# matyasosvath/hutoken

Hardware: AMD Instinct MI355X
Metric: GB/s input text encoded (GPT-2 vocab) at 1/2/4/8 GPUs; bit-exact ids (higher is better)
Workload: dtype u8

## Files before the change

hutoken_amd/csrc/hutk_kernels.hip:

```cpp
#include <hip/hip_runtime.h>

#include <type_traits>

#include "hutk_kdev.h"
#include "hutk_lab.h"

namespace hutk {

__device__ __noinline__ void cut_note_cold(uint32_t* noreal_bits, uint32_t* counters, uint32_t tile, unsigned long long mine,
                                                  uint32_t last16, uint32_t* cutpos) {
    if ((threadIdx.x & 63) != 0) return;
    if (mine == 0) {
        atomicOr(&noreal_bits[tile >> 5], 1u << (tile & 31));
        atomicAdd(&counters[CTR_NOREAL_TILES], 1u);
    } else {
        *cutpos = 1u + (uint32_t)(16 * (63 - __builtin_clzll(mine)) + 31 - __builtin_clz(last16 & 0xFFFFu));
    }
}

struct Win8 { uint32_t d[8]; };
__device__ __noinline__ uint32_t classify16_exact_cold(Win8 w, uint32_t dbits, uint32_t* tmp) {
#pragma unroll
    for (int i = 0; i < 8; i++) tmp[i] = w.d[i];
    return classify16_exact(*reinterpret_cast<const uint32_t(*)[8]>(tmp), dbits);
// ... 161 lines not shown
            if (X.arena_ws[a] == ws) return X.arena_n[a];
        int n = 0;
        for (int i = 0; i < nb; i++) n += !is_cont(X.sb[ws + LOOKBACK + i]);
        return n;
    };
    static_assert(LOOKBACK + TILE_BYTES + 3 + 4 * (wc::KEY_DWORDS + 1) <= WINDOW, "key reads inside the window");
    [[maybe_unused]] auto wc_key = [&](const Tile& X, int ws, int nb, uint32_t (&k)[wc::KEY_DWORDS]) {
        const int a = (ws + LOOKBACK) & ~3, o8 = 8 * ((ws + LOOKBACK) & 3);
        const uint32_t* sw = reinterpret_cast<const uint32_t*>(X.sb + a);
        uint32_t q[wc::KEY_DWORDS + 1];
#pragma unroll
        for (int j = 0; j <= wc::KEY_DWORDS; j++) q[j] = sw[j];
#pragma unroll
        for (int j = 0; j < wc::KEY_DWORDS; j++) k[j] = funnel_r(q[j + 1], q[j], o8);
        wc::make_key(k, nb);
    };
    [[maybe_unused]] bool learn_open = false;
    [[maybe_unused]] const uint32_t wc_shard = blockIdx.x & (wc::LIST_SHARDS - 1u), wc_shard_cap = W.wc_list_cap / wc::LIST_SHARDS;
    if constexpr (WCACHE && !ONE) {
        if (T.wc_on && W.wc_list_cap) {
            const uint32_t cnt = __hip_atomic_load(&T.wc_ctl[wc::ctl_count(wc_shard)], __ATOMIC_RELAXED, __HIP_MEMORY_SCOPE_AGENT);
            const uint32_t closed = __hip_atomic_load(&T.wc_ctl[wc::CTL_CLOSED], __ATOMIC_RELAXED, __HIP_MEMORY_SCOPE_AGENT);
            learn_open = __builtin_amdgcn_readfirstlane((int)(cnt < wc_shard_cap && closed == 0)) != 0;
        }
    }
    const int64_t t0 = tile * TILE_BYTES;
    const int64_t gw = t0 - LOOKBACK;
    const uint32_t* wmask32 = reinterpret_cast<const uint32_t*>(wmask16);
    const int64_t tile_end = (t0 + TILE_BYTES < A.n_bytes) ? t0 + TILE_BYTES : A.n_bytes;
    int64_t dfirst = 0;
    if constexpr (ONE) {
        if (threadIdx.x == 0) { *A.err = 0; W.noreal_bits[0] = 0; }
        if (threadIdx.x < N_COUNTERS) W.counters[threadIdx.x] = 0;
        if (A.status)
            for (int64_t d = threadIdx.x; d < A.n_docs; d += 64 * WAVES) A.status[d] = 0;
        if (tile_ok) {
            int64_t cnt = 0;
            for (int64_t d0 = 0; d0 <= A.n_docs; d0 += 64) {
                const int64_t d = d0 + lane;
                cnt += __popcll(__ballot(d <= A.n_docs && A.offsets[d] < gw));
            }
            dfirst = cnt;
            if (lane == 0) W.tile_first_doc[tile] = cnt;
        }
    } else {
        dfirst = tile_ok ? W.tile_first_doc[tile] : 0;
    }
    uint32_t own = 0;
    static_assert(WINDOW / 16 > 64 && WINDOW / 16 <= 128, "two chunks per lane");
    const bool whole = tile_ok && gw >= 0 && gw + WINDOW <= A.n_bytes;
    uint4 pre0 = make_uint4(0, 0, 0, 0), pre1 = pre0;
    if (whole) {
        pre0 = *reinterpret_cast<const uint4*>(A.bytes + gw + 16 * lane);
        if (lane < WINDOW / 16 - 64) pre1 = *reinterpret_cast<const uint4*>(A.bytes + gw + 16 * (lane + 64));
    }
    constexpr int DFA_CHUNKS = (dfa::TABLE_BYTES + 256) / 16;
    static_assert(DFA_CHUNKS <= 2 * 64 * WAVES || WAVES < 4, "two chunks of the automaton's table per thread");
    uint4 dfa0 = make_uint4(0, 0, 0, 0), dfa1 = dfa0;
    if (WAVES >= 4) {
        if ((int)threadIdx.x < DFA_CHUNKS) dfa0 = T.split_dfa[threadIdx.x];
        if ((int)threadIdx.x + 64 * WAVES < DFA_CHUNKS) dfa1 = T.split_dfa[threadIdx.x + 64 * WAVES];
    }
    int64_t pre_o = 0;
    if (tile_ok && !A.first_bits && dfirst + lane <= A.n_docs) pre_o = A.offsets[dfirst + lane];
    if (WAVES >= 4) {
        if ((int)threadIdx.x < DFA_CHUNKS) reinterpret_cast<uint4*>(&s_m.c)[threadIdx.x] = dfa0;
        if ((int)threadIdx.x + 64 * WAVES < DFA_CHUNKS) reinterpret_cast<uint4*>(&s_m.c)[threadIdx.x + 64 * WAVES] = dfa1;
    } else {
        for (int i = threadIdx.x; i < DFA_CHUNKS; i += 64 * WAVES) reinterpret_cast<uint4*>(&s_m.c)[i] = T.split_dfa[i];
    }
    if (!BYTE_MODE) {
        for (int i = threadIdx.x; i < 256; i += 64 * WAVES) {
            s_item_sym[i] = Sym<SymT>::narrow(T.item_sym[i]);
            const unsigned long long direct = __ballot(T.item_direct[i] != 0);
            if (lane == 0) {
                s_item_direct[i >> 5] = (uint32_t)direct;
                s_item_direct[(i >> 5) + 1] = (uint32_t)(direct >> 32);
            }
        }
    }
    if (threadIdx.x == 0) s_exc_cnt = 0;
    __syncthreads();
    uint32_t my_exc_off = 0;
    if (tile_ok) {
        HUTK_STAMP(0);

        if (whole) {
            *reinterpret_cast<uint4*>(sb + 16 * lane) = pre0;
            if (lane < WINDOW / 16 - 64) *reinterpret_cast<uint4*>(sb + 16 * (lane + 64)) = pre1;
        } else
        for (int c = lane; c < WINDOW / 16; c += 64) {
            const int64_t p = gw + 16 * c;
            if (p >= 0 && p + 16 <= A.n_bytes) {
                *reinterpret_cast<uint4*>(sb + 16 * c) = *reinterpret_cast<const uint4*>(A.bytes + p);
            } else {
                for (int k = 0; k < 16; k++) {
                    const int64_t q = p + k;
                    sb[16 * c + k] = (q >= 0 && q < A.n_bytes) ? A.bytes[q] : (uint8_t)0;
                }
            }
        }
        if (lane < WINDOW / 32 + 3) docm[lane] = 0;
        if (lane < NPOS / 32 + 2) { mergem[lane] = 0; excm[lane] = 0; livem[lane] = 0; }
        if (lane == 0) { s_arena_used = 0; s_extra = 0; me.cutpos = 0; }
        if (lane < ARENA_WORDS) { arena_ws[lane] = 0xFFFFu; arena_live[lane] = 0; }
        if (lane < 8) wmask16[64 + lane] = 0xFFFFu;
        wave_sync();

        if (A.first_bits) {
            if (lane < WINDOW / 32) {
                const int64_t g = gw + 32 * lane;
                const int64_t w = g >> 5;
                const uint32_t lo = w >= 0 ? A.first_bits[w] : 0u, hi = A.first_bits[w + 1];
                docm[lane] = (lo >> 16) | (hi << 16);
            }
        } else
        for (int64_t d = dfirst + lane; d <= A.n_docs; d += 64) {
            const int64_t o = d == dfirst + lane ? pre_o : A.offsets[d];
            if (o >= gw + WINDOW) break;
            const int li = (int)(o - gw);
            if (li >= 0) atomicOr(&docm[li >> 5], 1u << (li & 31));
        }
        wave_sync();
        HUTK_STAMP(1);

        const int kb = LOOKBACK + 16 * lane;
        Win w;
        {
            const uint64_t* src = reinterpret_cast<const uint64_t*>(sb + kb - 8);
            w.a = src[0]; w.b = src[1]; w.c = src[2]; w.d = src[3];
        }
        const uint32_t dbits = (uint32_t)bits64(docm, kb - 8);
        uint32_t flags;
        unsigned long long with_start;
        uint32_t last_real16;
        {
            const uint32_t dw[8] = {(uint32_t)w.a, (uint32_t)(w.a >> 32), (uint32_t)w.b, (uint32_t)(w.b >> 32),
                                    (uint32_t)w.c, (uint32_t)(w.c >> 32), (uint32_t)w.d, (uint32_t)(w.d >> 32)};
            bool exotic;
            if (A.word_bits) {
                flags = reinterpret_cast<const uint16_t*>(A.word_bits)[(t0 >> 4) + lane];
                exotic = false;
            } else {
                flags = classify16_dfa(dw, dbits, reinterpret_cast<const uint16_t*>(s_m.c.dfa), s_m.c.lut,
                                       &exotic);
            }
            if (exotic) {
                Win8 w8;
    #pragma unroll
                for (int i = 0; i < 8; i++) w8.d[i] = dw[i];
                flags = classify16_exact_cold(w8, dbits, reinterpret_cast<uint32_t*>(S) + 8 * lane);
            }
            with_start = __ballot(flags != 0);
            last_real16 = (uint32_t)__builtin_amdgcn_readlane((int)flags, 63 - __builtin_clzll((with_start & 0x0FFFFFFFFFFFFFFFull) | 1ull));
            if (T.seam_on && !A.word_bits) {
                const uint64_t K8 = 0x8080808080808080ull;
                uint64_t m0 = w.b & (w.b << 1) & (w.b << 2) & K8;
                uint64_t m1 = w.c & (w.c << 1) & (w.c << 2) & K8;
                if (m0 | m1) {
                    const uint64_t p0 = (w.b << 8) | (w.a >> 56), p1 = (w.c << 8) | (w.b >> 56);
                    for (; m0; m0 &= m0 - 1) {
                        const int sh = __builtin_ctzll(m0) - 7;
                        const uint32_t y = (uint32_t)(w.b >> sh) & 0xFFu, x = (uint32_t)(p0 >> sh) & 0xFFu;
                        const uint32_t sm = *reinterpret_cast<const uint32_t*>(s_m.c.dfa + dfa::seam_offset(x));
                        bool join = (sm >> (y & 31u)) & 1u;
                        if (!join) flags |= 1u << (sh >> 3);
                    }
                    for (; m1; m1 &= m1 - 1) {
                        const int sh = __builtin_ctzll(m1) - 7;
                        const uint32_t y = (uint32_t)(w.c >> sh) & 0xFFu, x = (uint32_t)(p1 >> sh) & 0xFFu;
                        const uint32_t sm = *reinterpret_cast<const uint32_t*>(s_m.c.dfa + dfa::seam_offset(x));
                        bool join = (sm >> (y & 31u)) & 1u;
                        if (!join) flags |= 1u << (8 + (sh >> 3));
                    }
                }
            }
        }
        {
            const int64_t valid = tile_end - (t0 + 16 * lane);
            const uint64_t lo = w.b, hi = w.c;
            const uint64_t K1 = 0x0101010101010101ull, K8 = 0x8080808080808080ull;
            uint64_t zlo = (lo - K1) & ~lo & K8, zhi = (hi - K1) & ~hi & K8;
            if (valid < 16) {
                const int v = valid < 0 ? 0 : (int)valid;
                zlo &= v >= 8 ? ~0ull : ((1ull << (8 * v)) - 1ull);
                zhi &= v <= 8 ? 0ull : ((1ull << (8 * (v - 8))) - 1ull);
            }
            if (zlo | zhi) raise(A.err, HUTK_E_NUL_BYTE);
        }
        {
            const unsigned long long sb_ = __ballot((flags & 0xFFFFu) != 0);
            const int l0 = sb_ ? __builtin_ctzll(sb_) : 0;
            const uint32_t f0 = (uint32_t)__builtin_amdgcn_readlane((int)flags, l0) & 0xFFFFu;
            if (lane == 0 && tile_ok) W.tile_first_start[tile] = sb_ ? (uint32_t)(16 * l0 + __builtin_ctz(f0)) : 0xFFFFu;
        }
        wmask16[lane] = (uint16_t)flags;
#if HUTK_PERTURB_VALU
        {
            uint32_t x = flags | 1u;
            for (int i = 0; i < HUTK_PERTURB_VALU / 4; i++) {
                x ^= x << 13; x ^= x >> 17;
                asm volatile("" : "+v"(x));
            }
            if (x == 0x9E3779B9u) raise(A.err, HUTK_E_MEMORY);
        }
#endif
        HUTK_STAMP(2);

        wave_sync();
        HUTK_STAMP(3);

        const int limit = (int)(tile_end - t0);
        own = flags;
        {
            const int lo = 16 * lane;
            if (lo >= limit) own = 0;
            else if (lo + 16 > limit) own &= (1u << (limit - lo)) - 1u;
        }
        if (!A.word_bits || !A.gap_bits) {
            const unsigned long long mine = with_start & ((1ull << ((limit + 15) >> 4)) - 1ull);
            if (mine == 0 || (with_start >> 60) == 0)
                cut_note_cold(W.noreal_bits, W.counters, (uint32_t)tile, mine, last_real16, &me.cutpos);
        }
        reinterpret_cast<uint16_t*>(livem)[lane] = (uint16_t)own;
        uint32_t rest = own;
        if constexpr (BYTE_MODE && !MULTI) {
            if (!A.word_bits && ONE) {
                constexpr int WORD_KEY = sizeof(SymT) == 2 ? WORD_KEY_BYTES_16 : WORD_KEY_BYTES_32;
                constexpr int KSH = sizeof(SymT) == 2 ? 16 : 32;
                const uint32_t f32 = flags | ((uint32_t)wmask16[lane + 1] << 16);
                uint32_t x = f32 >> 1;
                x |= x >> 1;
                x |= x >> 2;
                x |= x >> 4;
                x |= x >> (WORD_KEY - 8);
                uint32_t shorts = own & x;
                if (T.has_prefix) shorts &= ~(uint32_t)bits64(docm, 16 * lane + LOOKBACK);
                rest = own & ~shorts;
                uint32_t nS;
                uint32_t sidx = wave_excl_scan(__popc(shorts), lane, &nS);
                for (uint32_t r0 = 0; r0 < nS; r0 += 64) {
                    while (shorts && sidx - r0 < 64u) {
                        stage[sidx - r0] = (uint16_t)(16 * lane + __builtin_ctz(shorts));
                        shorts &= shorts - 1;
                        sidx++;
                    }
                    wave_sync();
                    if (r0 + lane < nS) {
                        const uint32_t ws = stage[lane];
                        uint32_t wb;
                        __builtin_memcpy(&wb, reinterpret_cast<const uint8_t*>(wmask16) + ((ws + 1u) >> 3), 4);
                        const uint32_t nb = 1u + (uint32_t)__builtin_ctz(wb >> ((ws + 1u) & 7u));
                        uint4 key;
                        __builtin_memcpy(&key, sb + LOOKBACK + ws, 16);
                        const uint32_t isym = T.item_sym[key.x & 0xFFu];
                        const uint64_t mlo = nb >= 8 ? ~0ull : ((1ull << (8 * nb)) - 1ull);
                        const uint64_t mhi = nb <= 8 ? 0ull : ((1ull << (8 * (nb - 8))) - 1ull);
                        const uint32_t k0 = key.x & (uint32_t)mlo, k1 = key.y & (uint32_t)(mlo >> 32);
                        const uint32_t k2 = key.z & (uint32_t)mhi, k3 = key.w & (uint32_t)(mhi >> 32);
                        bool done = nb == 1;
                        uint32_t sym = isym;
                        if (T.word_mask) {
                            const uint32_t wh = word_hash(k0, k1, k2, k3);
                            uint4 s1 = reinterpret_cast<const uint4*>(T.word_tab)[wh & T.word_mask];
                            uint4 s2 = reinterpret_cast<const uint4*>(T.word_tab)[word_slot2(wh, T.word_mask)];
                            asm volatile("" : "+v"(s1.x), "+v"(s2.x));
                            const uint32_t d1 = KSH == 32 ? 0u : (s1.w ^ k3) << (KSH & 31);
                            const uint32_t d2 = KSH == 32 ? 0u : (s2.w ^ k3) << (KSH & 31);
                            const bool hit1 = ((s1.x ^ k0) | (s1.y ^ k1) | (s1.z ^ k2) | d1) == 0;
                            const bool hit2 = ((s2.x ^ k0) | (s2.y ^ k1) | (s2.z ^ k2) | d2) == 0;
                            if (nb != 1 && (hit1 || hit2)) {
                                const uint32_t swd = hit1 ? s1.w : s2.w;
                                sym = KSH == 32 ? swd : swd >> (KSH & 31);
                                done = true;
                            }
                        }
                        if (done) {
                            S[ws] = Sym<SymT>::narrow(sym);
                        } else {
                            atomicOr(&mergem[ws >> 5], 1u << (ws & 31));
                        }
                    }
                    wave_sync();
                }
            }
        }
        uint32_t nW;
        const uint32_t wbase = wave_excl_scan(__popc(rest), lane, &nW);
        uint32_t widx = wbase;
        for (uint32_t r0 = 0; r0 < nW; r0 += 64) {
            while (rest && widx - r0 < 64u) {
                stage[widx - r0] = (uint16_t)(16 * lane + __builtin_ctz(rest));
                rest &= rest - 1;
                widx++;
            }
            wave_sync();
            if (r0 + lane < nW) {
                const int ws = stage[lane];
                const uint64_t nxt = bits64(wmask32, ws + 1) & 0x7FFFFFFFFFFFFFFFull;
                const int nb = nxt ? 1 + __builtin_ctzll(nxt) : 64;
                const bool known_end = nxt != 0 && (ws + nb < NPOS || t0 + ws + nb >= A.n_bytes);
                const bool docfirst = bit_at(docm, ws + LOOKBACK);
                const uint32_t b0 = sb[ws + LOOKBACK];
                const bool gap = A.gap_bits && ((A.gap_bits[(t0 + ws) >> 5] >> ((t0 + ws) & 31)) & 1u);
                const bool sp0 = A.alone_bits ? gbit(A.alone_bits, t0 + ws) : b0 == ' ';
                const bool pfx = !gap && T.has_prefix && docfirst && !sp0;
                bool exc = !gap && (!known_end || nb > LANE_MAX_BYTES || (BYTE_MODE && T.has_prefix && docfirst));
                if (MULTI && !gap && !exc) {
                    bool m = false;
                    for (int i = 0; i < nb; i++) {
// ... 70 lines not shown
                    done = hit1 || hit2;
                    const uint32_t sw = hit1 ? s1.w : s2.w;
                    if (done) S[ws] = Sym<SymT>::narrow(KSH == 32 ? sw : sw >> (KSH & 31));
                }
                if (probe_long) {
                    done = ((s1.x ^ k0) | (s1.y ^ k1) | (s1.z ^ k2) | (s1.w ^ k3) | (s2.x ^ k4) | (s2.y ^ k5) | (s2.z ^ k6)) == 0;
                    if (done) S[ws] = Sym<SymT>::narrow(s2.w);
                }
                int n = 0;
                SymT* Sdst = S + ws;
                int slot = -1;
                if (!BYTE_MODE && !exc && pfx) {
                    slot = (int)atomicAdd(&s_arena_used, 1u);
                    if (slot >= ARENA_WORDS ||
                        atomicAdd(&s_extra, (uint32_t)T.n_prefix) + T.n_prefix > (uint32_t)RUN_EXTRA) exc = true;
                    else {
                        Sdst = arenaS + slot * ARENA_W;
                        for (int i = 0; i < T.n_prefix && i < ARENA_W; i++) Sdst[i] = Sym<SymT>::narrow(T.prefix_syms[i]);
                        n = T.n_prefix;
                    }
                }
                const int n_cap = pfx ? ARENA_W : LANE_MAX_UNITS;
                if (!gap && !exc && !done) {
                    if (BYTE_MODE) {
                        n = nb;
                    } else {
                        const int lw = ws + LOOKBACK;
                        int i = 0;
                        while (i < nb) {
                            const uint32_t b = sb[lw + i];
                            int L = 1;
                            if (b >= 0x80u) {
                                L = (b >= 0xF0u) ? 4 : (b >= 0xE0u) ? 3 : (b >= 0xC0u) ? 2 : 1;
                                if (L == 1 || i + L > nb) { raise(A.err, HUTK_E_INVALID_UTF8); L = 1; }
                            }
                            uint32_t sym;
                            if ((s_item_direct[b >> 5] >> (b & 31u)) & 1u) sym = Sym<SymT>::widen(s_item_sym[b]);
                            else if (L == 1) sym = SYM_UNK;
                            else {
                                uint32_t packed = b | ((uint32_t)sb[lw + i + 1] << 8);
                                if (L > 2) packed |= (uint32_t)sb[lw + i + 2] << 16;
                                if (L > 3) packed |= (uint32_t)sb[lw + i + 3] << 24;
                                sym = char_lookup(T, packed);
                            }
                            if (n < n_cap) Sdst[n] = Sym<SymT>::narrow(sym);
                            n++;
                            i += L;
                        }
                    }
                    if (n > LANE_MAX_UNITS) exc = true;
                }
                if (gap) {
                    atomicAnd(&livem[ws >> 5], ~(1u << (ws & 31)));
                    done = true;
                } else if (done) {
                } else if (!BYTE_MODE && !exc && pfx) {
                    arena_ws[slot] = (uint16_t)ws;
                    arena_n[slot] = (uint16_t)n;
                    atomicAnd(&livem[ws >> 5], ~(1u << (ws & 31)));
                } else if (exc) {
                    atomicOr(&excm[ws >> 5], 1u << (ws & 31));
                    atomicAnd(&livem[ws >> 5], ~(1u << (ws & 31)));
                    done = true;
                } else if (n == 1) {
                    if (BYTE_MODE) S[ws] = Sym<SymT>::narrow(isym);
                    done = true;
                }
                if (!done) atomicOr(&mergem[ws >> 5], 1u << (ws & 31));
            }
            wave_sync();
        }
        HUTK_STAMP(4);
        {
            const uint32_t e16 = reinterpret_cast<const uint16_t*>(excm)[lane];
            if (__any(e16 != 0)) {
                uint32_t tot;
                (void)wave_excl_scan((uint32_t)__popc(e16), lane, &tot);
                uint32_t off = 0;
                if (lane == 0) off = atomicAdd(&s_exc_cnt, tot | (1u << 16));
                my_exc_off = (uint32_t)__builtin_amdgcn_readfirstlane((int)off);
            }
        }

        if constexpr (WCACHE) {
            if (T.wc_on) {
                uint32_t pend = reinterpret_cast<const uint16_t*>(mergem)[lane];
                uint32_t nP;
                uint32_t pidx = wave_excl_scan((uint32_t)__popc(pend), lane, &nP);
                for (uint32_t r0 = 0; r0 < nP; r0 += 64) {
                    while (pend && pidx - r0 < 64u) {
                        stage[pidx - r0] = (uint16_t)(16 * lane + __builtin_ctz(pend));
                        pend &= pend - 1;
                        pidx++;
                    }
                    wave_sync();
                    if (r0 + lane < nP) {
                        const int ws = stage[lane];
                        const int nb = word_units(me, ws);
                        if (nb >= wc::MIN_BYTES && nb <= wc::KEY_BYTES) {
                            uint32_t k[wc::KEY_DWORDS];
                            wc_key(me, ws, nb, k);
                            const uint4* line = T.wc_tab + (size_t)wc::bucket_of(wc::hash(k), T.wc_log2) * 8u;
                            uint4 a0 = line[0], a1 = line[1], b0 = line[4], b1 = line[5];
                            asm volatile("" : "+v"(a0.x), "+v"(a1.x), "+v"(b0.x), "+v"(b1.x));
                            const uint32_t s1[wc::KEY_DWORDS] = {a0.x, a0.y, a0.z, a0.w, a1.x, a1.y, a1.z, a1.w};
                            const uint32_t s2[wc::KEY_DWORDS] = {b0.x, b0.y, b0.z, b0.w, b1.x, b1.y, b1.z, b1.w};
                            const bool hit1 = wc::key_hit(s1, k), hit2 = wc::key_hit(s2, k);
                            if (hit1 || hit2) {
                                const uint4* sy = line + (hit1 ? 2 : 6);
                                const uint4 y0 = sy[0], y1 = sy[1];
                                const int n = wc::slot_n(hit1 ? a1.w : b1.w);
                                const uint32_t y[8] = {y0.x, y0.y, y0.z, y0.w, y1.x, y1.y, y1.z, y1.w};
#pragma unroll
                                for (int i = 0; i < wc::MAX_IDS; i++)
                                    if (i < n) S[ws + i] = (SymT)(y[i >> 1] >> (16 * (i & 1)));
                                const uint64_t lm = (uint64_t)(((1u << n) - 1u) & ~1u) << (ws & 31);
                                if ((uint32_t)lm) atomicOr(&livem[ws >> 5], (uint32_t)lm);
                                if ((uint32_t)(lm >> 32)) atomicOr(&livem[(ws >> 5) + 1], (uint32_t)(lm >> 32));
                                atomicAnd(&mergem[ws >> 5], ~(1u << (ws & 31)));
                            }
                        }
                    }
                    wave_sync();
                }
            }
        }
    }

#if HUTK_ABLATE_MERGE
    if (tile_ok) reinterpret_cast<uint16_t*>(mergem)[lane] = 0;
#endif
#if HUTK_PERTURB_SLEEP
    for (int i = 0; i < HUTK_PERTURB_SLEEP; i++) __builtin_amdgcn_s_sleep(127);
#endif
    [[maybe_unused]] bool first_epoch = true;
    for (;;) {
#if HUTK_MERGE_STAMPS
        if (first_epoch && tile_ok && W.prof && lane == 0)
            W.prof[tile * N_PHASE + 0] = (clock64() & ~3ll) | (long long)__builtin_amdgcn_s_getreg((1 << 11) | (4 << 6) | 4);
#endif
        if (threadIdx.x == 0) { pool_cnt[0] = 0; pool_cnt[1] = 0; pool_cnt[2] = FAST_TRIPS ? 2u : 0u; }
        __syncthreads();
        if (first_epoch && threadIdx.x == 0 && s_exc_cnt != 0) {
            const uint32_t cnt = s_exc_cnt;
            s_exc_base = atomicAdd(reinterpret_cast<unsigned long long*>(W.counters),
                                   ((unsigned long long)(cnt >> 16) << 32) | (unsigned long long)(cnt & 0xFFFFu));
        }
        if (first_epoch) HUTK_MSTAMP(1);
        uint32_t pending = 0;
        if (tile_ok) {
            pending = reinterpret_cast<const uint16_t*>(mergem)[lane];
            for (uint32_t m = pending; m; m &= m - 1) {
                const int j = __builtin_ctz(m);
                const int ws = 16 * lane + j;
                const int n = word_units(me, ws);
                const bool is_long = n > POOL_LONG;
                const uint32_t moff = atomicAdd(&pool_cnt[2], (uint32_t)n);
                if (moff + n > (uint32_t)M_ARENA) continue;
                const uint32_t idx = atomicAdd(&pool_cnt[is_long ? 0 : 1], 1u);
                if (idx < (uint32_t)(is_long ? POOL_LONG_CAP : POOL_CAP - POOL_LONG_CAP)) {
                    pool[is_long ? idx : POOL_CAP - 1 - idx] = (moff << 16) | (uint32_t)((wv << 10) | ws);
                    pending &= ~(1u << j);
                }
            }
            reinterpret_cast<uint16_t*>(mergem)[lane] = (uint16_t)pending;
        }
        if (first_epoch) HUTK_MSTAMP(2);
        __syncthreads();
        if (first_epoch) { HUTK_MSTAMP(3); HUTK_MSTAMP(4); }
        const uint32_t n_long = min(pool_cnt[0], (uint32_t)POOL_LONG_CAP);
        const uint32_t n_pool = n_long + min(pool_cnt[1], (uint32_t)(POOL_CAP - POOL_LONG_CAP));
        for (uint32_t base = 64u * wv; base < n_pool; base += 64u * WAVES) {
            const uint32_t wi = base + lane;
            bool have = wi < n_pool;
            const uint32_t entry = have ? (wi < n_long ? pool[wi] : pool[POOL_CAP - 1 - (wi - n_long)]) : 0u;
            Tile& X = L[(entry >> 10) & 63u];
            const int ws = entry & 1023;
            SymT* Sw = X.S + ws;
            SymT* Mw = s_m.g.m + (entry >> 16);
            int arena_slot = -1;
            int n = 0;
            if (have) {
                n = word_units(X, ws);
                if (!BYTE_MODE)
                    for (int a = 0; a < ARENA_WORDS; a++)
                        if (X.arena_ws[a] == ws) {
                            Sw = X.arenaS + a * ARENA_W;
                            Mw = X.arenaM + a * ARENA_W;
                            arena_slot = a;
                        }
            }
            if constexpr (FAST_TRIPS) {
                constexpr uint32_t NOKEY = 0xFFFFFFFFu;
                uint32_t live = 0, cand = 0, best = NOKEY;
                const uint32_t mw_lds = lds_addr(Mw);
                auto scan_key = [&](uint32_t c) -> uint32_t {
                    uint32_t b = NOKEY;
                    while (c) {
                        const uint32_t c1 = c & (c - 1), c2 = c1 & (c1 - 1), c3 = c2 & (c2 - 1);
                        const int i0 = ffbl_raw(c), i1 = ffbl_raw(c1), i2 = ffbl_raw(c2), i3 = ffbl_raw(c3);
                        uint32_t m0, m1, m2, m3;
                        lds_read4_u16(mw_lds + 2u * i0, mw_lds + 2u * i1, mw_lds + 2u * i2, mw_lds + 2u * i3, m0, m1, m2, m3);
                        const uint32_t k0 = (m0 << 5) | (uint32_t)i0, k1 = (m1 << 5) | (uint32_t)i1,
                                       k2 = (m2 << 5) | (uint32_t)i2, k3 = (m3 << 5) | (uint32_t)i3;
                        b = min(min(b, k0), min(min(k1, k2), k3));
                        c = c3 & (c3 - 1);
                    }
                    return b;
                };
                auto publish = [&]() {
                    if (!BYTE_MODE && arena_slot >= 0) {
                        X.arena_live[arena_slot] = live;
                        return;
                    }
                    const uint64_t lm = (uint64_t)(live & ~1u) << (ws & 31);
                    if ((uint32_t)lm) atomicOr(&X.livem[ws >> 5], (uint32_t)lm);
                    if ((uint32_t)(lm >> 32)) atomicOr(&X.livem[(ws >> 5) + 1], (uint32_t)(lm >> 32));
                };
                if (have && !BYTE_MODE) {
                    live = (n >= 32) ? 0xFFFFFFFFu : ((1u << n) - 1u);
                    for (int i0 = 0; i0 + 1 < n; i0 += 4) {
                        PairProbe pr[4];
                        uint32_t sy[5];
#pragma unroll
                        for (int j = 0; j < 5; j++) sy[j] = (i0 + j < n) ? (uint32_t)Sw[i0 + j] : 0u;
#pragma unroll
                        for (int j = 0; j < 4; j++) pr[j] = pair_issue(T, sy[j], sy[j + 1]);
#pragma unroll
                        for (int j = 0; j < 4; j++) {
                            const int i = i0 + j;
// ... 38 lines not shown
                    }
                    cand &= (1u << (n - 1)) - 1u;
                    best = scan_key(cand);
                }
                if (first_epoch && base == 64u * wv) HUTK_MSTAMP(4);
                const bool mine = have;
#if HUTK_MERGE_STAMPS
                long long ts_issue = 0, ts_scan = 0, ts_resolve = 0, ts_trips = 0;
#endif
                uint32_t again = 0;
                int p = 0;
                for (;;) {
#if HUTK_MERGE_STAMPS
                    const long long tt0 = clock64();
                    long long tt1 = tt0, tt2 = tt0;
#endif
                    have = have && (best != NOKEY || again != 0);
                    if (!__any(have)) break;
                    if (have) {
                        uint32_t merged;
                        if (again == 0) {
                            p = (int)(best & 31u);
                            merged = best >> 5;
                            const uint32_t above = live & ~((2u << p) - 1u);
                            const int q = __builtin_ctz(above);
                            Sw[p] = (SymT)merged;
                            live &= ~(1u << q);
                            cand &= ~((1u << q) | (1u << p));
                        } else {
                            merged = Sw[p];
                        }
                        const uint32_t rmask = live & ~((2u << p) - 1u);
                        const uint32_t lmask = live & ((1u << p) - 1u);
                        const int q2 = __builtin_ctz(rmask | 0x80000000u);
                        const int p0 = 31 - __builtin_clz(lmask | 1u);
                        const uint32_t sr = Sw[q2], sl = Sw[p0];
                        const uint32_t t1 = pair_mix(merged, sr), t2 = pair_mix(sl, merged);
                        uint32_t b1 = pair_bucket1(t1, T.pair_shift), b2 = pair_bucket1(t2, T.pair_shift);
                        if (again != 0) {
                            if (again & 1u) b1 = pair_bucket2(t1, T.pair_shift);
                            if (again & 2u) b2 = pair_bucket2(t2, T.pair_shift);
                        }
                        const uint4 e1 = T.pair_buckets[b1], e2 = T.pair_buckets[b2];
#if HUTK_MERGE_STAMPS
                        tt1 = clock64();
#endif
                        if (again == 0) {
                            cand &= ~(1u << p0);
                            best = scan_key(cand);
                        }
#if HUTK_MERGE_STAMPS
                        tt2 = clock64();
#endif
                        const uint32_t y1 = pair_match(e1, merged | ((sr & 0xFFFu) << 20), sr >> 12);
                        const uint32_t y2 = pair_match(e2, sl | ((merged & 0xFFFu) << 20), merged >> 12);
                        const uint32_t f1 = (e1.y >> 28) | ((e1.w >> 28) << 4), f2 = (e2.y >> 28) | ((e2.w >> 28) << 4);
                        const bool need1 = rmask != 0 && y1 == 0xFFFFFFFFu && !(again & 1u) && ((f1 >> (t1 & 7u)) & 1u);
                        const bool need2 = lmask != 0 && y2 == 0xFFFFFFFFu && !(again & 2u) && ((f2 >> (t2 & 7u)) & 1u);
                        if (need1 || need2) {
                            again |= (need1 ? 1u : 0u) | (need2 ? 2u : 0u);
                        } else {
                            again = 0;
                            uint32_t mr = (y1 >> 8) & 0xFFFFFu, ml = (y2 >> 8) & 0xFFFFFu;
                            mr = (rmask != 0 && mr != PAIR_ABSENT) ? mr : SYM_NONE;
                            ml = (lmask != 0 && ml != PAIR_ABSENT) ? ml : SYM_NONE;
                            Mw[p0] = (SymT)ml;
                            Mw[p] = (SymT)mr;
                            const bool hr = mr != SYM_NONE, hl = ml != SYM_NONE;
                            cand |= ((hr ? 1u : 0u) << p) | ((hl ? 1u : 0u) << p0);
                            const uint32_t kr = hr ? ((mr << 5) | (uint32_t)p) : NOKEY;
                            const uint32_t kl = hl ? ((ml << 5) | (uint32_t)p0) : NOKEY;
                            best = min(best, min(kr, kl));
                        }
                    }
#if HUTK_MERGE_STAMPS
                    {
                        const long long tt3 = clock64();
                        ts_issue += tt1 - tt0; ts_scan += tt2 - tt1; ts_resolve += tt3 - tt2; ts_trips++;
                    }
#endif
                }
#if HUTK_MERGE_STAMPS
                if (first_epoch && base == 64u * wv && tile_ok && W.prof && lane == 0) {
                    W.prof[tile * N_PHASE + 7] = ts_issue; W.prof[tile * N_PHASE + 8] = ts_scan;
                    W.prof[tile * N_PHASE + 9] = ts_resolve | (ts_trips << 40);
                }
#endif
                if (mine) {
                    publish();
                }
                if constexpr (WCACHE && !ONE) {
                    if (learn_open) {
                        const int nl = __popc(live);
                        const bool cand_ok = mine && wc::cacheable(n, nl);
                        const unsigned long long cb = __ballot(cand_ok);
                        if (cb) {
                            uint32_t first = 0;
                            if (lane == 0) first = atomicAdd(&T.wc_ctl[wc::ctl_count(wc_shard)], (uint32_t)__popcll(cb));
                            first = (uint32_t)__builtin_amdgcn_readfirstlane((int)first);
                            uint32_t at = first + (uint32_t)__popcll(cb & ((1ull << lane) - 1ull));
                            const bool room = at < wc_shard_cap;
                            at += wc_shard * wc_shard_cap;
                            if (cand_ok && room) {
                                uint32_t k[wc::KEY_DWORDS];
                                wc_key(X, ws, n, k);
                                k[7] = wc::with_n(k[7], nl);
                                uint32_t y[8], lv = live;
#pragma unroll
                                for (int i = 0; i < wc::MAX_IDS; i++) {
                                    uint32_t s = 0;
                                    if (lv) s = Sw[__builtin_ctz(lv)];
                                    lv &= lv - 1;
                                    if (i & 1) y[i >> 1] |= s << 16; else y[i >> 1] = s;
                                }
                                uint4* rec = W.wc_list + (size_t)at * 4u;
                                rec[0] = make_uint4(k[0], k[1], k[2], k[3]);
                                rec[1] = make_uint4(k[4], k[5], k[6], k[7]);
                                rec[2] = make_uint4(y[0], y[1], y[2], y[3]);
                                rec[3] = make_uint4(y[4], y[5], y[6], y[7]);
                            }
                        }
                    }
                }
                wave_sync();
            } else {
                uint32_t live = 0, cand = 0;
                uint32_t br = 0xFFFFFFFFu;
                int bp = 0;
                SymT bm = 0;
                if (have) {
                    live = (n >= 32) ? 0xFFFFFFFFu : ((1u << n) - 1u);
                    if (BYTE_MODE) {
                        const uint8_t* wb = X.sb + ws + LOOKBACK;
                        for (int i0 = 0; i0 < n; i0 += 16) {
                            typename Sym<SymT>::Pair e[16];
#pragma unroll
                            for (int j = 0; j < 16; j++) {
                                const int i = i0 + j;
                                const uint32_t b = (i < n) ? wb[i] : 0u, b2 = (i + 1 < n) ? wb[i + 1] : 0u;
                                e[j] = reinterpret_cast<const typename Sym<SymT>::Pair*>(T.bytepair)[b | (b2 << 8)];
                            }
#pragma unroll
                            for (int j = 0; j < 16; j++) {
                                const int i = i0 + j;
                                if (i < n) {
                                    const SymT mv = Sym<SymT>::pair_merged(e[j]);
                                    Sw[i] = Sym<SymT>::pair_sym(e[j]);
                                    Mw[i] = mv;
                                    if (i + 1 < n && mv != Sym<SymT>::NONE) cand |= 1u << i;
                                }
                            }
                        }
                    } else {
                        for (int i0 = 0; i0 + 1 < n; i0 += 4) {
                            PairProbe pr[4];
                            uint32_t sl[5];
#pragma unroll
                            for (int j = 0; j < 5; j++) sl[j] = (i0 + j < n) ? Sym<SymT>::widen(Sw[i0 + j]) : 0u;
#pragma unroll
                            for (int j = 0; j < 4; j++) pr[j] = pair_issue(T, sl[j], sl[j + 1]);
#pragma unroll
                            for (int j = 0; j < 4; j++) {
                                const int i = i0 + j;
                                if (i + 1 < n) {
                                    const uint32_t m = pair_resolve(T, pr[j], sl[j], sl[j + 1]);
                                    Mw[i] = Sym<SymT>::narrow(m);
                                    if (m != SYM_NONE) cand |= 1u << i;
                                }
// ... 394 lines not shown
    }
    if ((int64_t)W.tile_exc_first[tile] + (int64_t)nexc > W.cap_exc) continue;
    wave_sync();
    ExcRec* recs = W.exc + W.tile_exc_first[tile];
    for (uint32_t e = tid; e < nexc; e += GATHER_THREADS) {
        e_pos[e] = recs[e].wpos;
        e_cum[e + 1] = recs[e].tok_base < 0 ? 0u : recs[e].cnt;
        e_tok[e] = recs[e].tok_base;
        e_ws[e] = (uint16_t)(recs[e].ws - tile * TILE_BYTES);
    }
    wave_sync();
    {
        uint32_t carry = 0;
        for (uint32_t e0 = 0; e0 < nexc; e0 += GATHER_THREADS) {
            const uint32_t e = e0 + tid;
            const uint32_t v = e < nexc ? e_cum[e + 1] : 0u;
            uint32_t tot;
            const uint32_t before = wave_excl_scan(v, tid, &tot);
            if (e < nexc) e_cum[e + 1] = carry + before + v;
            carry += tot;
        }
        if (tid == 0) e_cum[0] = 0;
    }
    wave_sync();
    for (uint32_t k = tid; k < dense; k += GATHER_THREADS) {
        uint32_t lo = 0, hi = nexc;
        while (lo < hi) {
            const uint32_t mid = (lo + hi) >> 1;
            if (e_pos[mid] <= k) lo = mid + 1; else hi = mid;
        }
        A.ids_out[base + k + e_cum[lo]] = sym_to_id(T, run_sym(k));
    }
    for (uint32_t e = tid; e < nexc; e += GATHER_THREADS) recs[e].out_pos = base + e_pos[e] + e_cum[e];
    {
        const int64_t t0 = tile * TILE_BYTES;
        const int64_t t_end = (t0 + TILE_BYTES < A.n_bytes) ? t0 + TILE_BYTES : A.n_bytes;
        for (int64_t d = W.tile_first_doc[tile] + tid; d <= A.n_docs; d += GATHER_THREADS) {
            const int64_t o = A.offsets[d];
            if (o >= t_end) break;
            if (o < t0) continue;
            const uint32_t r = (uint32_t)(o - t0);
            uint32_t lo = 0, hi = nexc;
            while (lo < hi) {
                const uint32_t mid = (lo + hi) >> 1;
                if (e_ws[mid] < r) lo = mid + 1; else hi = mid;
            }
            A.out_offsets[d] = base + W.doc_tile_pos[d] + e_cum[lo];
        }
    }
    const uint32_t n_flat = e_cum[nexc];
    for (uint32_t k = tid; k < n_flat; k += GATHER_THREADS) {
        uint32_t lo = 0, hi = nexc;
        while (hi - lo > 1) {
            const uint32_t mid = (lo + hi) >> 1;
            if (e_cum[mid] <= k) lo = mid; else hi = mid;
        }
        A.ids_out[base + e_pos[lo] + k] = W.exc_tok[e_tok[lo] + (k - e_cum[lo])];
    }
    }
}

__device__ __forceinline__ void d_doc_off(const BatchArgs& A, const Workspace& W, int64_t vblock) {
    const int64_t d = vblock * blockDim.x + threadIdx.x;
    if (d > A.n_docs) return;
    const int64_t o = A.offsets[d];
    if (o >= A.n_bytes) {
        A.out_offsets[d] = W.tile_base[A.n_tiles];
        return;
    }
    const int64_t tile = o / TILE_BYTES;
    const int64_t v = W.tile_base[tile] + W.doc_tile_pos[d];
    if (W.tile_nexc[tile]) return;
    A.out_offsets[d] = v;
}


constexpr int LEARN_BLOCKS = 128;
static_assert(wc::LIST_SHARDS >= (uint32_t)LEARN_BLOCKS, "every d_learn workgroup has a sub-list (and so passes the loop's barriers)");
__device__ __forceinline__ void d_learn(const DevTables& T, const Workspace& W, uint32_t vblock, uint32_t vgrid) {
    __shared__ uint32_t s_cnt[3];
    __shared__ uint32_t s_count;
    uint32_t* const ctl = T.wc_ctl;
    const uint32_t shard_cap = W.wc_list_cap / wc::LIST_SHARDS;
    if (threadIdx.x < 3) s_cnt[threadIdx.x] = 0;
    uint32_t won = 0, dropped = 0;
    for (uint32_t shard = vblock; shard < wc::LIST_SHARDS; shard += vgrid) {
        __syncthreads();
        if (threadIdx.x == 0)
            s_count = min(__hip_atomic_load(&ctl[wc::ctl_count(shard)], __ATOMIC_RELAXED, __HIP_MEMORY_SCOPE_AGENT), shard_cap);
        __syncthreads();
        const uint32_t count = s_count;
        if (count == 0) continue;
        for (uint32_t i = threadIdx.x; i < count; i += blockDim.x) {
            const uint4* rec = W.wc_list + ((size_t)shard * shard_cap + i) * 4u;
            const uint4 r0 = rec[0], r1 = rec[1], r2 = rec[2], r3 = rec[3];
            const uint32_t k[wc::KEY_DWORDS] = {r0.x, r0.y, r0.z, r0.w, r1.x, r1.y, r1.z, r1.w};
            if (!wc::cacheable(wc::slot_nb(r1.w), wc::slot_n(r1.w))) continue;
            const uint32_t h = wc::hash(k), tag = wc::tag_of(k);
            const uint32_t slot0 = 2u * wc::bucket_of(h, T.wc_log2);
            bool placed_or_known = false;
            for (uint32_t sl = slot0; sl < slot0 + 2u && !placed_or_known; sl++) {
                const uint32_t old = atomicCAS(&T.wc_tags[sl], 0u, tag);
                if (old == 0u) {
                    uint4* dst = T.wc_tab + (size_t)sl * 4u;
                    dst[0] = r0; dst[1] = r1; dst[2] = r2; dst[3] = r3;
                    won++;
                }
                placed_or_known = old == 0u || old == tag;
            }
            if (!placed_or_known) dropped++;
        }
        if (threadIdx.x == 0) {
            atomicAdd(&s_cnt[0], count);
            __hip_atomic_store(&ctl[wc::ctl_count(shard)], 0u, __ATOMIC_RELAXED, __HIP_MEMORY_SCOPE_AGENT);
        }
    }
    if (won) atomicAdd(&s_cnt[1], won);
    if (dropped) atomicAdd(&s_cnt[2], dropped);
    __syncthreads();
    if (threadIdx.x == 0) {
        if (s_cnt[0]) {
            atomicAdd(&ctl[wc::CTL_B_LISTED], s_cnt[0]);
            if (s_cnt[1]) atomicAdd(&ctl[wc::CTL_B_WON], s_cnt[1]);
            if (s_cnt[2]) atomicAdd(&ctl[wc::CTL_B_DROPPED], s_cnt[2]);
            __threadfence();
        }
        if (atomicAdd(&ctl[wc::CTL_TICKET], 1u) == vgrid - 1u) {
            const uint32_t listed = atomicAdd(&ctl[wc::CTL_B_LISTED], 0u), placed = atomicAdd(&ctl[wc::CTL_B_WON], 0u);
            const uint32_t lost = atomicAdd(&ctl[wc::CTL_B_DROPPED], 0u);
            auto put = [&](int i, uint32_t v) { __hip_atomic_store(&ctl[i], v, __ATOMIC_RELAXED, __HIP_MEMORY_SCOPE_AGENT); };
            const uint32_t slots = 2u << T.wc_log2;
            const uint32_t entries = __hip_atomic_load(&ctl[wc::CTL_ENTRIES], __ATOMIC_RELAXED, __HIP_MEMORY_SCOPE_AGENT) + placed;
            put(wc::CTL_ENTRIES, entries);
            if ((uint64_t)entries * wc::CLOSE_DEN >= (uint64_t)slots * wc::CLOSE_NUM ||
                (lost > placed && (uint64_t)lost * wc::CLOSE_DROP_DIV >= slots))
                put(wc::CTL_CLOSED, 1u);
            put(wc::CTL_LAST, listed);
            put(wc::CTL_B_LISTED, 0u); put(wc::CTL_B_WON, 0u); put(wc::CTL_B_DROPPED, 0u);
            put(wc::CTL_TICKET, 0u);
        }
    }
}

constexpr int FINISH_EXC_BLOCKS = 2048;
template <typename RunT>
__global__ __launch_bounds__(64 * GATHER_WAVES) void k_finish(DevTables T, BatchArgs A, Workspace W, uint32_t g_gather, uint32_t g_doc) {
    const uint32_t b = blockIdx.x;
    if (b < g_gather) {
        d_gather<RunT>(T, A, W, (int64_t)b * GATHER_WAVES + (threadIdx.x >> 6));
    } else if (b < g_gather + FINISH_EXC_BLOCKS) {
        __shared__ __attribute__((aligned(16))) uint8_t lds_exc[cmax(GATHER_WAVES * ((gather_exc_lds(GATHER_EXC_SMALL) + 15) & ~(size_t)15), gather_exc_lds(GATHER_EXC_LDS))];
        if (W.counters[CTR_EXC_TILES] != 0) {
            const uint32_t wv = threadIdx.x >> 6;
            d_gather_exc<GATHER_EXC_SMALL, -1>(T, A, W, (b - g_gather) * GATHER_WAVES + wv, FINISH_EXC_BLOCKS * GATHER_WAVES,
                                               lds_exc + wv * ((gather_exc_lds(GATHER_EXC_SMALL) + 15) & ~(size_t)15));
            __syncthreads();
            if (wv == 0)
                for (uint32_t w4 = 0; w4 < (uint32_t)GATHER_WAVES; w4++)
                    d_gather_exc<GATHER_EXC_LDS, 1>(T, A, W, (b - g_gather) * GATHER_WAVES + w4, FINISH_EXC_BLOCKS * GATHER_WAVES, lds_exc);
        }
    } else if (b < g_gather + FINISH_EXC_BLOCKS + g_doc) {
        d_doc_off(A, W, (int64_t)(b - g_gather - FINISH_EXC_BLOCKS));
    } else {
        const uint32_t first = g_gather + FINISH_EXC_BLOCKS + g_doc;
        d_learn(T, W, b - first, gridDim.x - first);
    }
}

constexpr uint32_t CUT_MIN_RUN = (uint32_t)((MAX_WORD_BYTES + 1 - TILE_BYTES) / TILE_BYTES);
constexpr int CUT_THREADS = 1024;
__global__ __launch_bounds__(CUT_THREADS) void k_cut(DevTables T, BatchArgs A, Workspace W) {
    if (W.counters[CTR_NOREAL_TILES] < CUT_MIN_RUN) return;
    __shared__ EndsLds L;
    __shared__ uint32_t s_n_cuts;
    __shared__ int32_t s_vals[CUT_THREADS];
    uint32_t* const cut_doc = W.exc_quad;
    uint32_t* const cut_keep = W.exc_wave;
    const int tid = threadIdx.x, lane = tid & 63;
    if (tid == 0) s_n_cuts = 0;
    __syncthreads();
    if (tid < 64) {
        const int64_t n_words = (A.n_tiles + 31) / 32;
        auto bit = [&](int64_t t) -> bool { return t < A.n_tiles && ((W.noreal_bits[t >> 5] >> (t & 31)) & 1u); };
        int64_t last_doc = -1;
        uint32_t nc = 0;
        EndsWin cw;
        for (int64_t w0 = 0; w0 < n_words; w0 += 64) {
            const int64_t w = w0 + lane;
            const uint32_t bits = w < n_words ? W.noreal_bits[w] : 0u;
            const uint32_t prev = (w > 0 && w <= n_words) ? W.noreal_bits[w - 1] : 0u;
            const bool head = bits == 0xFFFFFFFFu && prev != 0xFFFFFFFFu;
            for (unsigned long long bal = __ballot(head); bal; bal &= bal - 1) {
                const int l = __builtin_ctzll(bal);
                {
                    const uint32_t pv = (uint32_t)__shfl((int)prev, l, 64);
                    const int64_t t_first = (w0 + l) * 32 - __builtin_clz(~pv);
                    int64_t t_end = (w0 + l) * 32;
                    while (bit(t_end)) {
                        if ((t_end & 31) == 0 && t_end + 32 <= A.n_tiles && W.noreal_bits[t_end >> 5] == 0xFFFFFFFFu) t_end += 32;
                        else t_end++;
                    }
                    if (t_end - t_first < (int64_t)CUT_MIN_RUN || t_first == 0) continue;
                    const int64_t tp = t_first - 1;
                    const uint32_t lr = W.tile_lastreal[tp];
                    const int64_t P = tp * TILE_BYTES + (int64_t)(lr & 0xFFFFu);
                    const int64_t d = doc_of(A, W, P, (uint32_t)tp), ds = A.offsets[d], de = A.offsets[d + 1];
                    if (d == last_doc) continue;
                    int64_t E = de;
                    if (t_end * TILE_BYTES < de) {
                        bool unused;
                        E = exc_word_end(T, A, t_end * TILE_BYTES - 1, d, ds, de, L.sb, L.scode, L.docm, lane, &unused, cw, false);
                        if (E > de) E = de;
                    }
                    if (E - P <= MAX_WORD_BYTES) continue;
                    uint32_t exc_ids = 0;
                    const uint32_t nexc = W.tile_nexc[tp], first = W.tile_exc_first[tp];
                    for (uint32_t e = lane; e < nexc; e += 64) {
                        const uint64_t idx = (uint64_t)first + e;
                        if ((int64_t)idx >= W.cap_exc) break;
                        const ExcRec r = W.exc[idx];
                        if (r.ws < P && r.tok_base >= 0) exc_ids += r.cnt;
                    }
                    for (int o = 32; o; o >>= 1) exc_ids += (uint32_t)__shfl_xor((int)exc_ids, o, 64);
                    const int64_t idpos = W.tile_base[tp] + (int64_t)(lr >> 16) + exc_ids;
                    const int64_t keep = idpos - A.out_offsets[d];
                    if (lane == 0) {
                        cut_doc[nc] = (uint32_t)d;
                        cut_keep[nc] = (uint32_t)keep;
                        if (A.status) A.status[d] = HUTK_DOC_WORD_TOO_LARGE;
                        raise(A.err, HUTK_E_WORD_TOO_LARGE);
                    }
                    nc++;
                    last_doc = d;
                }
            }
        }
        if (lane == 0) s_n_cuts = nc;
    }
    __threadfence();
    __syncthreads();
    const uint32_t nc = s_n_cuts;
    if (nc == 0) return;
    int64_t shift = 0, seg_begin = 0, doc_begin = 0;
    const int64_t total = A.out_offsets[A.n_docs];
    for (uint32_t c = 0; c <= nc; c++) {
        int64_t seg_end, doc_end, removed = 0;
        if (c < nc) {
            const int64_t d = cut_doc[c], a = A.out_offsets[d], b = A.out_offsets[d + 1];
// ... 171 lines not shown
```

hutoken_amd/csrc/hutk_lab.h:

```cpp
#pragma once
#ifndef HUTK_PERTURB_VALU
#define HUTK_PERTURB_VALU 0
#endif
#ifndef HUTK_PERTURB_MEM
#define HUTK_PERTURB_MEM 0
#endif
#ifndef HUTK_PERTURB_SLEEP
#define HUTK_PERTURB_SLEEP 0
#endif
#ifndef HUTK_ABLATE_MERGE
#define HUTK_ABLATE_MERGE 0
#endif
#ifndef HUTK_MERGE_STAMPS
#define HUTK_MERGE_STAMPS 0
#endif
#ifndef HUTK_LAB_LDS_PAD
#define HUTK_LAB_LDS_PAD 0
#endif
#ifndef HUTK_PT_PROF
#define HUTK_PT_PROF 0
#endif
#ifndef HUTK_PT_PERTURB_VALU
#define HUTK_PT_PERTURB_VALU 0
#endif
#ifndef HUTK_PT_PERTURB_SLEEP
#define HUTK_PT_PERTURB_SLEEP 0
#endif
#ifndef HUTK_PT_MARKS
#define HUTK_PT_MARKS 0
#endif
#define HUTK_STAMP_AT(k)                                                       \
    do {                                                                       \
        if (W.prof && lane == 0) W.prof[tile * N_PHASE + (k)] = clock64();     \
    } while (0)
#if HUTK_MERGE_STAMPS
#define HUTK_STAMP(k) do {} while (0)
#define HUTK_MSTAMP(k) do { if (tile_ok) HUTK_STAMP_AT(k); } while (0)
#else
#define HUTK_STAMP(k) HUTK_STAMP_AT(k)
#define HUTK_MSTAMP(k) do {} while (0)
#endif
```

Measured before the change: 281.4.

## Skip merge epoch loop via block vote when no words pending; reorder learn blocks

```diff
diff --git a/hutoken_amd/csrc/hutk_kernels.hip b/hutoken_amd/csrc/hutk_kernels.hip
--- a/hutoken_amd/csrc/hutk_kernels.hip
+++ b/hutoken_amd/csrc/hutk_kernels.hip
@@ -267,8 +267,14 @@
     if (threadIdx.x == 0) s_exc_cnt = 0;
     __syncthreads();
     uint32_t my_exc_off = 0;
+#if HUTK_MERGE_STAMPS
+    long long ts_tile = 0;
+#endif
     if (tile_ok) {
         HUTK_STAMP(0);
+#if HUTK_MERGE_STAMPS
+        ts_tile = clock64();
+#endif
 
         if (whole) {
             *reinterpret_cast<uint4*>(sb + 16 * lane) = pre0;
@@ -410,7 +416,7 @@
         reinterpret_cast<uint16_t*>(livem)[lane] = (uint16_t)own;
         uint32_t rest = own;
         if constexpr (BYTE_MODE && !MULTI) {
-            if (!A.word_bits && ONE) {
+            if (!A.word_bits && (ONE || (HUTK_LAB_SLIM_ROUNDS && WCACHE))) {
                 constexpr int WORD_KEY = sizeof(SymT) == 2 ? WORD_KEY_BYTES_16 : WORD_KEY_BYTES_32;
                 constexpr int KSH = sizeof(SymT) == 2 ? 16 : 32;
                 const uint32_t f32 = flags | ((uint32_t)wmask16[lane + 1] << 16);
@@ -647,6 +653,9 @@
             }
         }
 
+#if HUTK_MERGE_STAMPS
+        const long long ts_6a = clock64();
+#endif
         if constexpr (WCACHE) {
             if (T.wc_on) {
                 uint32_t pend = reinterpret_cast<const uint16_t*>(mergem)[lane];
@@ -667,13 +676,22 @@
                             wc_key(me, ws, nb, k);
                             const uint4* line = T.wc_tab + (size_t)wc::bucket_of(wc::hash(k), T.wc_log2) * 8u;
                             uint4 a0 = line[0], a1 = line[1], b0 = line[4], b1 = line[5];
+#if HUTK_LAB_PROBE_ONE_TRIP
+                            uint4 ya0 = line[2], ya1 = line[3], yb0 = line[6], yb1 = line[7];
+                            asm volatile("" : "+v"(a0.x), "+v"(a1.x), "+v"(b0.x), "+v"(b1.x), "+v"(ya0.x), "+v"(ya1.x), "+v"(yb0.x), "+v"(yb1.x));
+#else
                             asm volatile("" : "+v"(a0.x), "+v"(a1.x), "+v"(b0.x), "+v"(b1.x));
+#endif
                             const uint32_t s1[wc::KEY_DWORDS] = {a0.x, a0.y, a0.z, a0.w, a1.x, a1.y, a1.z, a1.w};
                             const uint32_t s2[wc::KEY_DWORDS] = {b0.x, b0.y, b0.z, b0.w, b1.x, b1.y, b1.z, b1.w};
                             const bool hit1 = wc::key_hit(s1, k), hit2 = wc::key_hit(s2, k);
                             if (hit1 || hit2) {
+#if HUTK_LAB_PROBE_ONE_TRIP
+                                const uint4 y0 = hit1 ? ya0 : yb0, y1 = hit1 ? ya1 : yb1;
+#else
                                 const uint4* sy = line + (hit1 ? 2 : 6);
                                 const uint4 y0 = sy[0], y1 = sy[1];
+#endif
                                 const int n = wc::slot_n(hit1 ? a1.w : b1.w);
                                 const uint32_t y[8] = {y0.x, y0.y, y0.z, y0.w, y1.x, y1.y, y1.z, y1.w};
 #pragma unroll
@@ -690,6 +708,17 @@
                 }
             }
         }
+#if HUTK_MERGE_STAMPS
+        if (W.prof) {
+            const bool left = __any(reinterpret_cast<const uint16_t*>(mergem)[lane] != 0);
+            const long long now = clock64();
+            if (lane == 0) {
+                W.prof[tile * N_PHASE + 9] = 0;
+                W.prof[tile * N_PHASE + 7] = ts_tile;
+                W.prof[tile * N_PHASE + 8] = ((ts_6a - ts_tile) & 0xFFFFFFll) | (((now - ts_6a) & 0xFFFFFFll) << 24) | ((long long)left << 48);
+            }
+        }
+#endif
     }
 
 #if HUTK_ABLATE_MERGE
@@ -699,18 +728,32 @@
     for (int i = 0; i < HUTK_PERTURB_SLEEP; i++) __builtin_amdgcn_s_sleep(127);
 #endif
     [[maybe_unused]] bool first_epoch = true;
+    constexpr bool VOTE_ENTRY = WCACHE && !ONE && !HUTK_LAB_PLAIN_ENTRY;
+    auto claim_exc = [&]() {
+        const uint32_t cnt = s_exc_cnt;
+        s_exc_base = atomicAdd(reinterpret_cast<unsigned long long*>(W.counters),
+                               ((unsigned long long)(cnt >> 16) << 32) | (unsigned long long)(cnt & 0xFFFFu));
+    };
     for (;;) {
 #if HUTK_MERGE_STAMPS
         if (first_epoch && tile_ok && W.prof && lane == 0)
             W.prof[tile * N_PHASE + 0] = (clock64() & ~3ll) | (long long)__builtin_amdgcn_s_getreg((1 << 11) | (4 << 6) | 4);
 #endif
         if (threadIdx.x == 0) { pool_cnt[0] = 0; pool_cnt[1] = 0; pool_cnt[2] = FAST_TRIPS ? 2u : 0u; }
-        __syncthreads();
-        if (first_epoch && threadIdx.x == 0 && s_exc_cnt != 0) {
-            const uint32_t cnt = s_exc_cnt;
-            s_exc_base = atomicAdd(reinterpret_cast<unsigned long long*>(W.counters),
-                                   ((unsigned long long)(cnt >> 16) << 32) | (unsigned long long)(cnt & 0xFFFFu));
-        }
+        if (VOTE_ENTRY && first_epoch) {
+            if (!__syncthreads_or(tile_ok && reinterpret_cast<const uint16_t*>(mergem)[lane] != 0)) {
+                HUTK_MSTAMP(1); HUTK_MSTAMP(2); HUTK_MSTAMP(3); HUTK_MSTAMP(4); HUTK_MSTAMP(5);
+                if (s_exc_cnt != 0) {
+                    if (threadIdx.x == 0) claim_exc();
+                    __syncthreads();
+                }
+                HUTK_MSTAMP(6);
+                break;
+            }
+        } else {
+            __syncthreads();
+        }
+        if (first_epoch && threadIdx.x == 0 && s_exc_cnt != 0) claim_exc();
         if (first_epoch) HUTK_MSTAMP(1);
         uint32_t pending = 0;
         if (tile_ok) {
@@ -915,8 +958,7 @@
                 }
 #if HUTK_MERGE_STAMPS
                 if (first_epoch && base == 64u * wv && tile_ok && W.prof && lane == 0) {
-                    W.prof[tile * N_PHASE + 7] = ts_issue; W.prof[tile * N_PHASE + 8] = ts_scan;
-                    W.prof[tile * N_PHASE + 9] = ts_resolve | (ts_trips << 40);
+                    W.prof[tile * N_PHASE + 9] = (ts_issue + ts_scan + ts_resolve) | (ts_trips << 40);
                 }
 #endif
                 if (mine) {
@@ -1477,6 +1519,7 @@
     __shared__ uint32_t s_count;
     uint32_t* const ctl = T.wc_ctl;
     const uint32_t shard_cap = W.wc_list_cap / wc::LIST_SHARDS;
+    if (__hip_atomic_load(&ctl[wc::CTL_CLOSED], __ATOMIC_RELAXED, __HIP_MEMORY_SCOPE_AGENT) != 0) return;
     if (threadIdx.x < 3) s_cnt[threadIdx.x] = 0;
     uint32_t won = 0, dropped = 0;
     for (uint32_t shard = vblock; shard < wc::LIST_SHARDS; shard += vgrid) {
@@ -1539,8 +1582,13 @@
 
 constexpr int FINISH_EXC_BLOCKS = 2048;
 template <typename RunT>
-__global__ __launch_bounds__(64 * GATHER_WAVES) void k_finish(DevTables T, BatchArgs A, Workspace W, uint32_t g_gather, uint32_t g_doc) {
-    const uint32_t b = blockIdx.x;
+__global__ __launch_bounds__(64 * GATHER_WAVES) __attribute__((amdgpu_num_sgpr(100))) void k_finish(DevTables T, BatchArgs A, Workspace W, uint32_t g_gather, uint32_t g_doc) {
+    const uint32_t g_learn = gridDim.x - (g_gather + FINISH_EXC_BLOCKS + g_doc);
+    if (blockIdx.x < g_learn) {
+        d_learn(T, W, blockIdx.x, g_learn);
+        return;
+    }
+    const uint32_t b = blockIdx.x - g_learn;
     if (b < g_gather) {
         d_gather<RunT>(T, A, W, (int64_t)b * GATHER_WAVES + (threadIdx.x >> 6));
     } else if (b < g_gather + FINISH_EXC_BLOCKS) {
@@ -1554,11 +1602,8 @@
                 for (uint32_t w4 = 0; w4 < (uint32_t)GATHER_WAVES; w4++)
                     d_gather_exc<GATHER_EXC_LDS, 1>(T, A, W, (b - g_gather) * GATHER_WAVES + w4, FINISH_EXC_BLOCKS * GATHER_WAVES, lds_exc);
         }
-    } else if (b < g_gather + FINISH_EXC_BLOCKS + g_doc) {
+    } else {
         d_doc_off(A, W, (int64_t)(b - g_gather - FINISH_EXC_BLOCKS));
-    } else {
-        const uint32_t first = g_gather + FINISH_EXC_BLOCKS + g_doc;
-        d_learn(T, W, b - first, gridDim.x - first);
     }
 }
 
diff --git a/hutoken_amd/csrc/hutk_lab.h b/hutoken_amd/csrc/hutk_lab.h
--- a/hutoken_amd/csrc/hutk_lab.h
+++ b/hutoken_amd/csrc/hutk_lab.h
@@ -16,6 +16,15 @@
 #endif
 #ifndef HUTK_LAB_LDS_PAD
 #define HUTK_LAB_LDS_PAD 0
+#endif
+#ifndef HUTK_LAB_PLAIN_ENTRY
+#define HUTK_LAB_PLAIN_ENTRY 0
+#endif
+#ifndef HUTK_LAB_PROBE_ONE_TRIP
+#define HUTK_LAB_PROBE_ONE_TRIP 0
+#endif
+#ifndef HUTK_LAB_SLIM_ROUNDS
+#define HUTK_LAB_SLIM_ROUNDS 0
 #endif
 #ifndef HUTK_PT_PROF
 #define HUTK_PT_PROF 0
```

Measured after the change: 281.4, median of 2. About the same (+0.0%).
